# rbitr/llm.f90

Hardware: AMD Instinct MI355X
Metric: tokens/sec TinyLlama-1.1B decode (higher is better)
Workload: dtype f32; 1 GPU; tinyllama f32 decode, greedy, positions 6..1140 (./llm -n 1140 -t 0); consumer=logits to host + host argmax (llmk_forward), parallelism=single GPU, seed=20260928

## Files before the change

### include/llmk.h

```cpp
#ifndef LLMK_H
#define LLMK_H

#include <stddef.h>
#include <stdint.h>

#ifdef __cplusplus
extern "C" {
#endif

#define LLMK_TYPE_F32 0
#define LLMK_TYPE_F16 1
#define LLMK_TYPE_Q4_0 2
#define LLMK_TYPE_Q6_K 14

#define LLMK_TOKEN_EMBEDDING_TABLE 0
#define LLMK_RMS_ATT_WEIGHT 1
#define LLMK_RMS_FFN_WEIGHT 2
#define LLMK_WQKV 3
#define LLMK_WO 4
#define LLMK_W13 5
#define LLMK_W2 6
#define LLMK_RMS_FINAL_WEIGHT 7
#define LLMK_WCLS 8
#define LLMK_N_TENSORS 9

#define LLMK_FLAG_NO_GRAPH 1
#define LLMK_FLAG_TIMINGS 2
#define LLMK_FLAG_MULTI_KERNEL 4

#define LLMK_OK 0
#define LLMK_E_ARG 1
#define LLMK_E_SHAPE 2
#define LLMK_E_SIZE 3
#define LLMK_E_TYPE 4
#define LLMK_E_STATE 5
#define LLMK_E_NODEVICE 6
#define LLMK_E_NOMEM 7
#define LLMK_E_TIMEOUT 8
#define LLMK_E_COMM 9
#define LLMK_E_VERIFY 10
#define LLMK_E_NONFINITE 11
#define LLMK_E_HIP 1000

// ... 30 lines not shown
int llmk_tp_read_partial(llmk_ctx *ctx, float *out);
int llmk_tp_write_partial(llmk_ctx *ctx, const float *in);
int llmk_tp_read_logits(llmk_ctx *ctx, float *out_slice);

int llmk_upload(llmk_ctx *ctx, int tensor_id, const void *host, size_t nbytes, int ggml_type);

int llmk_upload_rows(llmk_ctx *ctx, int tensor_id, int layer, int row_offset, int rows, const void *host,
                     size_t nbytes, int ggml_type);

int llmk_set_tensor_type(llmk_ctx *ctx, int tensor_id, int ggml_type);
int llmk_set_rms_eps(llmk_ctx *ctx, float eps);

int llmk_set_rope_freqs(llmk_ctx *ctx, const float *freqs, int n);

int llmk_forward(llmk_ctx *ctx, int token, int pos, float *logits_out);

int llmk_prefill(llmk_ctx* ctx, const int* tokens, int n, int pos0, float* logits_out);

int llmk_score(llmk_ctx *ctx, const int *tokens, int n, int pos0, const int *targets, float *logprob_out, int *argmax_out,
               float *logits_out);

int llmk_forward_greedy(llmk_ctx *ctx, int token, int pos, int *next_token);

typedef void (*llmk_token_fn)(int index, int token, void *user);
int llmk_decode_greedy(llmk_ctx *ctx, int token, int pos0, int n, int *ids_out, llmk_token_fn on_token, void *user);

int llmk_forward_sample(llmk_ctx *ctx, int token, int pos, float temperature, uint64_t seed, int *next_token);
int llmk_decode_sample(llmk_ctx *ctx, int token, int pos0, int n, float temperature, uint64_t seed,
                       int *ids_out, llmk_token_fn on_token, void *user);

// ... 103 lines not shown
```

### llm.f90_amd/csrc/llmk.hip

```cpp
#include "../../include/llmk.h"
#include "kernels.h"
#include "token_kernel.h"
#include "prefill.h"
#include "batch.h"
#include "tp_p2p.h"

#include <rccl/rccl.h>

#include <algorithm>
#include <vector>

#include <float.h>
#include <math.h>
#include <stdio.h>
#include <stdlib.h>
#include <string.h>
#include <new>

using namespace llmk;

extern "C" int llmk_create_tp(const llmk_config* cfg, int tp_rank, int tp_size, llmk_ctx** out);
static int q16_build(llmk_ctx* c);

#define HIPCHK(expr)                                          \
// ... 62 lines not shown
    unsigned* d_tp_bad = nullptr;
    TpPeers peers = {};
    void* ipc_mapped[TP_MAX_RANKS] = {};
    bool p2p = false;
    float* d_part = nullptr;
    TensorDesc gdesc[LLMK_N_TENSORS];
    TensorDesc desc[LLMK_N_TENSORS];
    DevTensor t[LLMK_N_TENSORS];
    float *d_kc = nullptr, *d_vc = nullptr;
    float *d_x = nullptr, *d_q = nullptr, *d_xb = nullptr, *d_hb = nullptr, *d_logits = nullptr, *d_rope = nullptr;
    int *d_tokpos = nullptr, *d_next = nullptr;
    int* h_tokpos = nullptr;
    float* h_logits = nullptr;
    float* h_logits_dev = nullptr;
    bool tk_direct = true;
    TkNext* h_next = nullptr;
    TkDevWords* dev_words() const { return tk_words_behind<TkDevWords>(d_logits, V); }
    TkHostWords* host_words() const { return tk_words_behind<TkHostWords>(h_logits, V); }
    TkHostWords* host_words_dev() const { return tk_words_behind<TkHostWords>(h_logits_dev, V); }
    hipStream_t stream = nullptr;
    hipGraphExec_t graph[TAIL_COUNT][2] = {};
    llmk_sample_params* h_samp = nullptr;
    DevShadow<llmk_sample_params> samp_dev = {{}, true};
    llmk_filter_params* h_filt = nullptr;
    DevShadow<llmk_filter_params> filt_dev;
    int* d_hist = nullptr;
    int* d_pen_cnt = nullptr;
    llmk_penalty_params* d_pen = nullptr;
    llmk_penalty_params* h_pen = nullptr;
    llmk_logprob_record *d_lp = nullptr, *h_lp = nullptr;
// ... 265 lines not shown
    }
    return launch_gemv_t<EPI_STORE, true>(c->t[LLMK_WCLS].type, c->stream, a, c->n_cu);
}
hipError_t launch_embed(llmk_ctx* c) {
    hipLaunchKernelGGL(embed_kernel, dim3((c->E + 255) / 256), dim3(256), 0, c->stream,
                       (const float*)c->t[LLMK_TOKEN_EMBEDDING_TABLE].data, c->d_tokpos, c->d_x, c->E);
    return hipGetLastError();
}

#define HIPRET(expr)                     \
    do {                                 \
        hipError_t e_ = (expr);          \
        if (e_ != hipSuccess) return e_; \
    } while (0)

struct TkGreedy { int gflags = 0, id_index = 0; };
template <class TK>
hipError_t launch_token_kernel_t(llmk_ctx* c, bool direct, const TkGreedy& g) {
    TokenArgs a;
    a.gflags = g.gflags | ((TK_DEBUG && getenv("LLMK_TK_NOSYNC")) ? TKG_NOSYNC : 0);
    a.emb = (const float*)c->t[LLMK_TOKEN_EMBEDDING_TABLE].data;
    a.rms = (const float*)c->t[LLMK_RMS_ATT_WEIGHT].data;
    a.wqkv = TK::Q4 ? c->q16[LLMK_WQKV] : c->t[LLMK_WQKV].data;
    a.wo = TK::Q4 ? c->q16[LLMK_WO] : c->t[LLMK_WO].data;
    a.w13 = TK::Q4 ? c->q16[LLMK_W13] : c->t[LLMK_W13].data;
    a.w2 = TK::Q4 ? c->q16[LLMK_W2] : c->t[LLMK_W2].data;
    a.wcls = (TK::Q4 && !TK::CLSQ6) ? c->q16[LLMK_WCLS] : c->t[LLMK_WCLS].data;
    a.kc = c->d_kc;
    a.vc = c->d_vc;
    a.rope = c->d_rope;
    a.tokpos = (direct || g.gflags) ? nullptr : c->d_tokpos;
    a.tok_imm = (g.gflags & TKG_CAND_IN) ? g.id_index : c->h_tokpos[0];
    a.pos_imm = c->h_tokpos[1];
    a.serial_imm = c->h_tokpos[2];
    a.g_qkv = c->d_gran;
    a.logits = direct ? c->h_logits_dev : c->d_logits;
    a.err = &c->dev_words()->err;
    a.herr = (direct || g.gflags) ? &c->host_words_dev()->err : nullptr;
    a.zeros = c->d_zeros;
#ifdef LLMK_TK_DEBUG
    a.trace = c->d_trace;
#endif
    a.L = c->L;
    a.S = c->S;
    a.eps = c->eps;
    const dim3 grid((TK_DEBUG && c->tk_short_grid) ? TK_NCU - 1 : TK_NCU);
    if (g.gflags) hipLaunchKernelGGL((token_kernel<TK, true>), grid, dim3(TK_THREADS), c->tk_lds, c->stream, a);
    else hipLaunchKernelGGL((token_kernel<TK>), grid, dim3(TK_THREADS), c->tk_lds, c->stream, a);
    return hipGetLastError();
}
#ifndef LLMK_TK_EXTRA_SHAPES
#define LLMK_TK_EXTRA_SHAPES(X)
#endif
// ... 39 lines not shown
        return LLMK_OK;
    const size_t lds = ((size_t)TkLds<TK>::ATT_S + 2 * (size_t)c->S * sizeof(float) + 15) & ~(size_t)15;
    c->tk_lds = lds < 96 * 1024 ? 96 * 1024 : lds;
    if (c->tk_lds > 160 * 1024) return LLMK_OK;
    HIPCHK(hipFuncSetAttribute((const void*)token_kernel<TK>, hipFuncAttributeMaxDynamicSharedMemorySize, (int)c->tk_lds));
    HIPCHK(hipFuncSetAttribute((const void*)token_kernel<TK, true>, hipFuncAttributeMaxDynamicSharedMemorySize, (int)c->tk_lds));
    int per_cu = 0;
    HIPCHK(hipOccupancyMaxActiveBlocksPerMultiprocessor(&per_cu, token_kernel<TK>, TK_THREADS, c->tk_lds));
    if (per_cu < 1 || (long long)per_cu * c->n_cu < TK_NCU) return LLMK_OK;
    static_assert(tk_qsc_front<TK>() == (size_t)TK::QKV + 3 * (size_t)TK::E + TK::H + (size_t)TK::NH * (TkAttPlan<TK>::PMAX - 1) * (TK::HS + 2),
                  "tk_qsc_front: the attention parts are TkAttPlan's");
    const size_t ngran = tk_qsc_front<TK>() + TK_QSC_GRANULES;
    c->tk_ngran = ngran;
    if (!c->d_gran) HIPCHK(dev_alloc(&c->d_gran, ngran * sizeof(unsigned long long)));
    if (!c->d_zeros) HIPCHK(dev_alloc(&c->d_zeros, (size_t)TK_NCU * TK_WAVES * 1024));
    if (TK_DEBUG && getenv("LLMK_TK_TRACE")) HIPCHK(dev_alloc(&c->d_trace, (size_t)TK_NCU * TK_TRACE_N * 8));
    HIPCHK(hipMemset(c->d_gran, 0, ngran * sizeof(unsigned long long)));
    HIPCHK(hipMemset(c->d_zeros, 0, (size_t)TK_NCU * TK_WAVES * 1024));
    c->use_tk = true;
    c->tk_shape = id;
    return LLMK_OK;
}

int tk_setup_all(llmk_ctx* c) {
    if ((c->cfg.flags & (LLMK_FLAG_MULTI_KERNEL | LLMK_FLAG_TIMINGS)) || c->n_cu != TK_NCU || c->tp_size != 1 || c->tk_retired) return LLMK_OK;
    int rc = LLMK_OK;
    for (int i = 0; i < TK_NSHAPES && rc == LLMK_OK; ++i) rc = tk_table[i].setup(c, i + 1);
    return rc;
}

__global__ void bump_serial_kernel(int* tokpos) { tokpos[2] += 1; }
// ... 173 lines not shown
            if (g) { hipGraphExecDestroy(g); g = nullptr; }
}
int build_graph(llmk_ctx* c, TailMode tail, hipGraphExec_t* out) {
    hipGraph_t g = nullptr;
    HIPCHK(hipStreamBeginCapture(c->stream, hipStreamCaptureModeThreadLocal));
    hipError_t e = enqueue_token(c, tail, false);
    hipError_t e2 = hipStreamEndCapture(c->stream, &g);
    if (e != hipSuccess) { if (g) hipGraphDestroy(g); return LLMK_E_HIP + (int)e; }
    HIPCHK(e2);
    e = hipGraphInstantiate(out, g, nullptr, nullptr, 0);
    hipGraphDestroy(g);
    HIPCHK(e);
    return LLMK_OK;
}

int check_ready(llmk_ctx* c) {
    if (!c) return LLMK_E_ARG;
    for (int i = 0; i < LLMK_N_TENSORS; ++i)
        if (!c->t[i].uploaded) return LLMK_E_STATE;
    if (c->use_tk && tk_table[c->tk_shape - 1].q4 && c->q16_dirty) return q16_build(c);
    return LLMK_OK;
}

constexpr int TK_RANGE_LIMIT = 4;
bool tk_inject_timeout(int pos) {
    const char* at = TK_DEBUG ? getenv("LLMK_TK_INJECT_TIMEOUT") : nullptr;
    return at && atoi(at) == pos;
}
int tk_clear_err(llmk_ctx* c) {
    HIPCHK(hipMemsetAsync(&c->dev_words()->err, 0, sizeof(unsigned), c->stream));
    HIPCHK(hipStreamSynchronize(c->stream));
    c->host_words()->err = 0;
// ... 83 lines not shown
            return LLMK_OK;
        }
        rc = tk_retire(c, err, pos);
        if (rc) return rc;
    }
    return LLMK_E_TIMEOUT;
}
int run_token(llmk_ctx* c, int token, int pos, TailMode tail) {
    const bool filt = tail == TAIL_FILTER || tail == TAIL_PENALTY, samp = tail == TAIL_SAMPLE;
    if (filt) c->filt_dev.invalidate();
    if (samp) c->samp_dev.invalidate();
    const int rc = run_token_pass(c, token, pos, tail);
    if (rc == LLMK_OK && filt) c->filt_dev.confirm(*c->h_filt);
    if (rc == LLMK_OK && samp) c->samp_dev.confirm(*c->h_samp);
    return rc;
}

#ifndef LLMK_PF_H_STEP1
#define LLMK_PF_H_STEP1 1.00
#define LLMK_PF_H_STEP2 1.32
#define LLMK_PF_HQ_STEP1 1.20
#define LLMK_PF_HQ_STEP2 1.92
#endif
struct PfPlan { int nr, nk, total, U, grid; };
PfPlan pf_plan(const llmk_ctx* c, int rows, int K, int T = PF_TMAX, int wt = -1) {
    if (wt < 0) wt = c->cfg.weight_type;
    static const double step_f32[2] = {2.45, 4.25}, step_h[2] = {LLMK_PF_H_STEP1, LLMK_PF_H_STEP2}, step_hq[2] = {LLMK_PF_HQ_STEP1, LLMK_PF_HQ_STEP2};
    static const double step_q8[2] = {LLMK_PF_HQ_STEP1, LLMK_PF_HQ_STEP2 * 0.925};
    static const double step_q6[2] = {LLMK_PF_HQ_STEP1 * 1.3, LLMK_PF_HQ_STEP2 * 1.3};
    const bool q6 = wt == LLMK_TYPE_Q6_K;
// ... 396 lines not shown
    HIPCHK(hipMemsetAsync(c->pf_flag, 0, sizeof(unsigned), c->stream));
    HIPCHK(hipStreamSynchronize(c->stream));
    pf_teardown(c);
    c->pf_hm = false;
    int rc = pf_setup(c);
    if (rc) return rc;
    rc = again();
    if (!for_good) pf_teardown(c);
    return rc;
}

}

extern "C" {

int llmk_version(void) { return 406; }

const char* llmk_strerror(int code) {
    switch (code) {
        case LLMK_OK: return "ok";
        case LLMK_E_ARG: return "llmk: bad argument";
        case LLMK_E_SHAPE: return "llmk: unsupported model shape";
        case LLMK_E_SIZE: return "llmk: byte count does not match tensor size";
        case LLMK_E_TYPE: return "llmk: unsupported ggml tensor type";
        case LLMK_E_STATE: return "llmk: forward called before all weights were uploaded";
        case LLMK_E_NODEVICE: return "llmk: no usable HIP device (there is no CPU fallback)";
        case LLMK_E_NOMEM: return "llmk: out of memory";
        case LLMK_E_TIMEOUT: return "llmk: device-side exchange timed out (persistent kernel not fully resident?)";
        case LLMK_E_COMM: return "llmk: tensor-parallel communicator missing or RCCL error";
        case LLMK_E_VERIFY: return "llmk: uploaded weights did not arrive intact on the device (three attempts)";
        case LLMK_E_NONFINITE: return "llmk: no finite logit at this position (the greedy or sampled pick has no answer)";
// ... 82 lines not shown
    CK(dev_alloc(&c->d_vc, kvn * sizeof(float)));
    CK(dev_alloc(&c->d_x, (size_t)E * sizeof(float)));
    CK(dev_alloc(&c->d_q, (size_t)E * sizeof(float)));
    CK(dev_alloc(&c->d_xb, (size_t)E * sizeof(float)));
    CK(dev_alloc(&c->d_hb, (size_t)H * sizeof(float)));
    CK(dev_alloc(&c->d_part, (size_t)E * sizeof(float)));
    const size_t logits_bytes = (size_t)V * sizeof(float) + sizeof(TkDevWords);
    CK(dev_alloc(&c->d_logits, logits_bytes));
    CK(dev_alloc(&c->d_rope, (size_t)(hs / 2) * sizeof(float)));
    CK(dev_alloc(&c->d_tokpos, 4 * sizeof(int)));
    CK(dev_alloc(&c->d_next, 2 * sizeof(int)));
    CK(hipHostMalloc(&c->h_tokpos, 4 * sizeof(int), hipHostMallocDefault));
    CK(hipHostMalloc(&c->h_logits, (size_t)V * sizeof(float) + sizeof(TkHostWords) + (size_t)S * sizeof(int), hipHostMallocMapped));
    CK(hipHostGetDevicePointer((void**)&c->h_logits_dev, c->h_logits, 0));
    c->tk_direct = !(getenv("LLMK_TK_DIRECT") && getenv("LLMK_TK_DIRECT")[0] == '0');
    CK(hipHostMalloc(&c->h_next, sizeof(TkNext), hipHostMallocDefault));
    CK(hipHostMalloc(&c->h_samp, sizeof(llmk_sample_params), hipHostMallocDefault));
    CK(hipHostMalloc(&c->h_filt, sizeof(llmk_filter_params), hipHostMallocDefault));
    CK(hipStreamCreateWithFlags(&c->stream, hipStreamNonBlocking));
    for (int i = 0; i < 8; ++i) CK(hipEventCreate(&c->ev[i]));
    if (rc == LLMK_OK) rc = tk_setup_all(c);
    if (rc == LLMK_OK) {
        g_prepare = true;
        hipError_t pe = launch_qkv(c, 0);
        if (pe == hipSuccess) pe = launch_attn(c, 0);
        if (pe == hipSuccess) pe = launch_wo(c, 0);
        if (pe == hipSuccess) pe = launch_w13(c, 0);
        if (pe == hipSuccess) pe = launch_w2(c, 0);
        if (pe == hipSuccess) pe = launch_cls(c);
        g_prepare = false;
// ... 220 lines not shown
        if (rc) return rc;
    }
    return LLMK_OK;
}

int llmk_upload_rows(llmk_ctx* c, int tid, int layer, int row_offset, int rows, const void* host, size_t nbytes,
                     int ggml_type) {
    if (!c || !host || tid < 0 || tid >= LLMK_N_TENSORS) return LLMK_E_ARG;
    const TensorDesc& g = c->gdesc[tid];
    DevTensor& t = c->t[tid];
    const int nl = g.layered ? c->L : 1;
    if (layer < 0 || layer >= nl || row_offset < 0 || rows <= 0 || row_offset + rows > g.rows) return LLMK_E_ARG;
    if (ggml_type != t.type) return LLMK_E_TYPE;
    if (nbytes != (size_t)rows * row_bytes_for(ggml_type, g.K)) return LLMK_E_SIZE;
    HIPCHK(hipSetDevice(c->cfg.device));
    if (c->tp_size > 1) return upload_rows_sharded(c, tid, layer, row_offset, rows, (const uint8_t*)host, ggml_type);
    const size_t pitch = row_bytes_for(ggml_type, g.K);
    return upload_block(c, tid, layer, row_offset, rows, (const uint8_t*)host, pitch, 0, pitch);
}

int llmk_upload(llmk_ctx* c, int tid, const void* host, size_t nbytes, int ggml_type) {
    if (!c || !host || tid < 0 || tid >= LLMK_N_TENSORS) return LLMK_E_ARG;
    const TensorDesc& g = c->gdesc[tid];
    const int nl = g.layered ? c->L : 1;
    if (ggml_type != c->t[tid].type) return LLMK_E_TYPE;
    const size_t per_layer = (size_t)g.rows * row_bytes_for(ggml_type, g.K);
    if (nbytes != per_layer * nl) return LLMK_E_SIZE;
    c->t[tid].rows_uploaded = 0;
    c->t[tid].uploaded = false;
    for (int l = 0; l < nl; ++l) {
        int rc = llmk_upload_rows(c, tid, l, 0, g.rows, (const char*)host + (size_t)l * per_layer, per_layer, ggml_type);
        if (rc) return rc;
    }
    return LLMK_OK;
}

int llmk_set_tensor_type(llmk_ctx* c, int tid, int ggml_type) {
    if (!c || tid != LLMK_WCLS) return LLMK_E_ARG;
    if (ggml_type != LLMK_TYPE_F32 && ggml_type != LLMK_TYPE_F16 && ggml_type != LLMK_TYPE_Q4_0 && ggml_type != LLMK_TYPE_Q6_K) return LLMK_E_TYPE;
    DevTensor& t = c->t[tid];
    if (t.type == ggml_type) return LLMK_OK;
    const TensorDesc& d = c->desc[tid];
    const int kalign = ggml_type == LLMK_TYPE_Q6_K ? Q6K_WEIGHTS : ggml_type == LLMK_TYPE_Q4_0 ? 32 : ggml_type == LLMK_TYPE_F16 ? 8 : 4;
    if (d.K % kalign) return LLMK_E_SHAPE;
    HIPCHK(hipSetDevice(c->cfg.device));
    HIPCHK(hipStreamSynchronize(c->stream));
    if (t.data) HIPCHK(hipFree(t.data));
    if (c->pf_ready) pf_teardown(c);
    t.data = nullptr;
    t.type = ggml_type;
    t.uploaded = false;
    t.rows_uploaded = 0;
    const size_t rows = (size_t)d.rows * (d.layered ? c->L : 1);
    t.row_bytes = dev_row_bytes(ggml_type, d.K);
    HIPCHK(dev_alloc(&t.data, rows * t.row_bytes + TENSOR_SLACK));
    HIPCHK(hipMemset(t.data, 0, rows * t.row_bytes + TENSOR_SLACK));
    if (c->q16[tid]) { HIPCHK(hipFree(c->q16[tid])); c->q16[tid] = nullptr; }
    c->q16_dirty = true;
    if (c->use_tk) {
        c->use_tk = false;
        drop_graphs(c);
    }
    { const int rc = tk_setup_all(c); if (rc) return rc; }
    g_prepare = true;
    const hipError_t pe = launch_cls(c);
    g_prepare = false;
    if (pe == hipErrorInvalidValue) return LLMK_E_SHAPE;
    HIPCHK(pe);
    return LLMK_OK;
}

int llmk_set_rms_eps(llmk_ctx* c, float eps) {
    if (!c || !(eps > 0.f) || !(eps < 1.f)) return LLMK_E_ARG;
    HIPCHK(hipSetDevice(c->cfg.device));
    HIPCHK(hipStreamSynchronize(c->stream));
    c->eps = eps;
    drop_graphs(c);
    return LLMK_OK;
}

int llmk_set_rope_freqs(llmk_ctx* c, const float* freqs, int n) {
    if (!c || !freqs || n != c->hs / 2) return LLMK_E_ARG;
    HIPCHK(hipSetDevice(c->cfg.device));
    HIPCHK(hipMemcpy(c->d_rope, freqs, (size_t)n * sizeof(float), hipMemcpyHostToDevice));
    return LLMK_OK;
}

int llmk_forward(llmk_ctx* c, int token, int pos, float* logits_out) {
    if (!c || !logits_out) return LLMK_E_ARG;
    int rc = run_token(c, token, pos, TAIL_LOGITS);
    if (rc) return rc;
    memcpy(logits_out, c->h_logits, (size_t)c->V * sizeof(float));
    return LLMK_OK;
}

int llmk_prefill(llmk_ctx* c, const int* tokens, int n, int pos0, float* logits_out) {
    if (!c || !tokens || !logits_out || n < 1 || pos0 < 1 || pos0 + n - 1 > c->S) return LLMK_E_ARG;
    int rc = check_ready(c);
    if (rc) return rc;
    for (int i = 0; i < n; ++i)
        if (tokens[i] < 1 || tokens[i] > c->V) return LLMK_E_ARG;
    if (!pf_eligible(c)) {
        for (int i = 0; i < n; ++i) {
            rc = run_token(c, tokens[i], pos0 + i, TAIL_LOGITS);
            if (rc) return rc;
        }
        memcpy(logits_out, c->h_logits, (size_t)c->V * sizeof(float));
// ... 272 lines not shown
                if (on_token) on_token(done, ids_out[done], user);
                ++done;
                continue;
            }
            const hipError_t q = hipStreamQuery(c->stream);
            if (q == hipSuccess) { if (ids[done] == 0) break; continue; }
            if (q != hipErrorNotReady) return LLMK_E_HIP + (int)q;
        }
        HIPCHK(hipStreamSynchronize(c->stream));
        for (; done < n && ids[done] != 0; ++done) {
            ids_out[done] = ids[done];
            if (on_token) on_token(done, ids_out[done], user);
        }
        const unsigned err = c->h_next->err;
        if (err == 0 && done == n) {
            for (int i = 0; lp && i < n; ++i) logprob_deliver(c, lp, i, pos0 + i - 1);
            return LLMK_OK;
        }
        rc = tk_range_only(err) ? tk_clear_err(c) : tk_retire(c, err, pos0 + done);
        if (rc) return rc;
        if (done > 0) token = ids_out[done - 1];
        c->tk_short_grid = false;
    }
    for (int i = done; i < n; ++i) {
        rc = run_token(c, token, pos0 + i, tail);
        if (rc) return rc;
        if (c->h_next->id < 1 || c->h_next->id > c->V) return LLMK_E_NONFINITE;
        token = ids_out[i] = c->h_next->id;
        if (lp) c->h_lp[pos0 + i - 1] = c->h_lp[c->S];
        if (on_token) on_token(i, token, user);
// ... 107 lines not shown
    *c->h_lp_top = (unsigned)top_n;
    HIPCHK(hipMemcpyAsync(c->d_logits, logits, (size_t)c->V * sizeof(float), hipMemcpyHostToDevice, c->stream));
    HIPCHK(copy_logprob_top(c));
    HIPCHK(enqueue_logprob(c, c->d_logits, nullptr, nullptr, 0, token, c->d_lp + c->S));
    HIPCHK(hipMemcpyAsync(c->h_lp + c->S, c->d_lp + c->S, sizeof(llmk_logprob_record), hipMemcpyDeviceToHost, c->stream));
    HIPCHK(hipStreamSynchronize(c->stream));
    logprob_deliver(c, &lp, 0, c->S);
    return LLMK_OK;
}
int llmk_set_history(llmk_ctx* c, const int* tokens, int n, int pos0) {
    if (!c || !tokens || n < 1 || pos0 < 1 || pos0 + n - 1 > c->S) return LLMK_E_ARG;
    for (int i = 0; i < n; ++i)
        if (tokens[i] < 0 || tokens[i] > c->V) return LLMK_E_ARG;
    const int rc = pen_setup(c);
    if (rc) return rc;
    HIPCHK(hipMemcpyAsync(c->d_hist + (pos0 - 1), tokens, (size_t)n * sizeof(int), hipMemcpyHostToDevice, c->stream));
    HIPCHK(hipStreamSynchronize(c->stream));
    return LLMK_OK;
}
int llmk_get_history(llmk_ctx* c, int* tokens_out, int n, int pos0) {
    if (!c || !tokens_out || n < 1 || pos0 < 1 || pos0 + n - 1 > c->S) return LLMK_E_ARG;
    const int rc = pen_setup(c);
    if (rc) return rc;
    HIPCHK(hipMemcpyAsync(tokens_out, c->d_hist + (pos0 - 1), (size_t)n * sizeof(int), hipMemcpyDeviceToHost, c->stream));
    HIPCHK(hipStreamSynchronize(c->stream));
    return LLMK_OK;
}

static_assert(LLMK_MAX_BATCH == PF_TMAX, "a batch's rows are the rows of one prefill pass");
constexpr size_t bd_attn_smem(int hs) { return ((size_t)BD_WAVES * 16 * hs + 2 * BD_WAVES * 16) * sizeof(float); }

static void batch_free(llmk_batch* b) {
    void* dev[] = {b->d_kc, b->d_vc, b->d_rows, b->d_tok, b->d_out, b->d_logits, b->d_po, b->d_pml, b->d_next, b->d_filt, b->d_out2, b->d_err, b->d_ids,
                   b->d_hist, b->d_pen_cnt, b->d_pen, b->d_raw, b->d_lp, b->d_lp_top, b->d_pk, b->d_pv, b->d_first, b->d_colmap, b->d_xpo, b->d_xpml};
    for (void* p : dev)
        if (p) hipFree(p);
    void* host[] = {b->h_rows, b->h_tok, b->h_filt, b->h_out, b->h_err, b->h_pen, b->h_lp, b->h_lp_top, b->h_first, b->h_colmap};
    for (void* p : host)
// ... 503 lines not shown
    if (pe == hipSuccess) pe = hipStreamSynchronize(c->stream);
    float ms = 0.f;
    if (pe == hipSuccess) pe = hipEventElapsedTime(&ms, e0, e1);
    hipEventDestroy(e0);
    if (e1) hipEventDestroy(e1);
    HIPCHK(hipMemsetAsync(c->pf_flag, 0, sizeof(unsigned), c->stream));
    HIPCHK(hipStreamSynchronize(c->stream));
    if (pe != hipSuccess) return LLMK_E_HIP + (int)pe;
    *avg_ms = ms / (float)iters;
    return LLMK_OK;
}

int llmk_reset(llmk_ctx* c) {
    if (!c) return LLMK_E_ARG;
    HIPCHK(hipSetDevice(c->cfg.device));
    const size_t kvn = (size_t)c->L * c->S * c->KVl * sizeof(float);
    HIPCHK(hipMemsetAsync(c->d_kc, 0, kvn, c->stream));
    HIPCHK(hipMemsetAsync(c->d_vc, 0, kvn, c->stream));
    HIPCHK(hipMemsetAsync(&c->dev_words()->err, 0, sizeof(unsigned), c->stream));
    HIPCHK(tk_qsc_clear(c, c->stream));
    if (c->d_hist) {
        HIPCHK(hipMemsetAsync(c->d_hist, 0, (size_t)c->S * sizeof(int), c->stream));
        HIPCHK(hipMemsetAsync(c->d_pen_cnt, 0, (size_t)c->V * sizeof(int), c->stream));
    }
    HIPCHK(hipStreamSynchronize(c->stream));
    c->host_words()->err = 0;
    c->h_next->err = 0;
    for (int i = 0; i < 5; ++i) c->times[i] = 0.f;
    return LLMK_OK;
}
// ... 133 lines not shown
    int rc = check_ready(c);
    if (rc) return -rc;
    if (!pf_shape_ok(c)) return LLMK_CLS_NONE;
    auto setup = [&]() -> int {
        HIPCHK(hipSetDevice(c->cfg.device));
        return pf_setup(c, true);
    };
    if ((rc = setup()) != LLMK_OK) return -rc;
    if (sc_plan(c, rows).R > 0) return LLMK_CLS_GEMM;
    return c->t[LLMK_WCLS].type == LLMK_TYPE_Q6_K ? LLMK_CLS_ROWS : LLMK_CLS_NONE;
}

int llmk_peek(llmk_ctx* c, int which, int layer, int pos, float* out, int n) {
    if (!c || !out || n <= 0) return LLMK_E_ARG;
    HIPCHK(hipSetDevice(c->cfg.device));
    const float* src = nullptr;
    int len = 0;
    switch (which) {
        case 0: src = c->d_x; len = c->E; break;
        case 1: src = c->d_q; len = c->Eq; break;
        case 2: src = c->d_xb; len = c->Eq; break;
        case 3: src = c->d_hb; len = c->Hl; break;
        case 4:
        case 5:
            if (layer < 0 || layer >= c->L || pos < 1 || pos > c->S) return LLMK_E_ARG;
            src = (which == 4 ? c->d_kc : c->d_vc) + ((size_t)layer * c->S + (pos - 1)) * c->KVl;
            len = c->KVl;
            break;
#ifdef LLMK_PF_TRACE
        case 7: src = c->pf[0].HB; len = PF_TMAX * c->H; break;
// ... 294 lines not shown
        if (ncclCommCount(c->comm, &n) != ncclSuccess) return -LLMK_E_COMM;
        return n;
    }
    if (c->p2p) {
        int n = 0;
        for (int r = 0; r < c->tp_size; ++r) n += c->peers.inbox[r] != nullptr;
        return n;
    }
    return 1;
}

int llmk_destroy(llmk_ctx* c) {
    if (!c) return LLMK_E_ARG;
    if (c->n_batches > 0) return LLMK_E_STATE;
    hipSetDevice(c->cfg.device);
    if (c->stream) hipStreamSynchronize(c->stream);
    if (c->comm) ncclCommDestroy(c->comm);
    for (int r = 0; r < TP_MAX_RANKS; ++r)
        if (c->ipc_mapped[r]) hipIpcCloseMemHandle(c->ipc_mapped[r]);
    if (c->d_inbox) hipFree(c->d_inbox);
    if (c->d_tp_bad) hipFree(c->d_tp_bad);
    drop_graphs(c);
    for (int i = 0; i < LLMK_N_TENSORS; ++i) {
        if (c->t[i].data && !c->t[i].alias) hipFree(c->t[i].data);
    }
    pf_teardown(c);
    sc_teardown(c);
    void* dev[] = {c->d_kc, c->d_vc, c->d_x, c->d_q, c->d_xb, c->d_hb, c->d_logits, c->d_rope, c->d_tokpos, c->d_next,
                   c->d_gran, c->d_zeros, c->d_trace, c->d_part, c->d_hist, c->d_pen_cnt, c->d_pen, c->d_lp, c->d_lp_raw};
    for (void* p : dev)
        if (p) hipFree(p);
    for (int b = 0; b < 2; ++b) {
        if (c->up_stage[b]) hipHostFree(c->up_stage[b]);
        if (c->up_tmp[b]) hipFree(c->up_tmp[b]);
        if (c->up_done[b]) hipEventDestroy(c->up_done[b]);
    }
    if (c->up_acc) hipFree(c->up_acc);
    for (int i = 0; i < LLMK_N_TENSORS; ++i)
        if (c->q16[i]) hipFree(c->q16[i]);
    if (c->h_tokpos) hipHostFree(c->h_tokpos);
    if (c->h_logits) hipHostFree(c->h_logits);
    if (c->h_next) hipHostFree(c->h_next);
    if (c->h_samp) hipHostFree(c->h_samp);
    if (c->h_filt) hipHostFree(c->h_filt);
    if (c->h_pen) hipHostFree(c->h_pen);
    if (c->h_lp) hipHostFree(c->h_lp);
    if (c->h_lp_top) hipHostFree(c->h_lp_top);
    for (int i = 0; i < 8; ++i)
        if (c->ev[i]) hipEventDestroy(c->ev[i]);
    if (c->stream) hipStreamDestroy(c->stream);
    delete c;
    return LLMK_OK;
}

}
```

### llm.f90_amd/llmk.py

```python
from __future__ import annotations

import ctypes as C
import os
import subprocess

import numpy as np

_HERE = os.path.dirname(os.path.abspath(__file__))
LIB_PATH = os.environ.get("LLMK_LIB") or os.path.join(_HERE, "csrc", "libllmk.so")

TENSOR_IDS = {
    "token_embedding_table": 0, "rms_att_weight": 1, "rms_ffn_weight": 2, "wqkv": 3, "wo": 4, "w13": 5, "w2": 6,
    "rms_final_weight": 7, "wcls": 8,
}
FLAG_NO_GRAPH, FLAG_TIMINGS, FLAG_MULTI_KERNEL = 1, 2, 4
SYMBOLS = ["llmk_create", "llmk_create_tp", "llmk_tp_unique_id", "llmk_tp_init_comm", "llmk_tp_p2p_handle", "llmk_tp_p2p_connect",
           "llmk_tp_p2p_connect_local", "llmk_tp_p2p_selftest", "llmk_tp_p2p_stress", "llmk_tp_p2p_disable", "llmk_tp_begin", "llmk_tp_segment",
           "llmk_tp_read_partial", "llmk_tp_write_partial", "llmk_tp_read_logits", "llmk_upload", "llmk_upload_rows",
           "llmk_set_rope_freqs", "llmk_set_tensor_type", "llmk_set_rms_eps", "llmk_forward", "llmk_prefill", "llmk_forward_greedy", "llmk_decode_greedy",
           "llmk_forward_sample", "llmk_decode_sample", "llmk_forward_sample_ex", "llmk_decode_sample_ex", "llmk_sample_logits", "llmk_set_history", "llmk_get_history",
           "llmk_forward_sample_pen", "llmk_decode_sample_pen", "llmk_sample_logits_pen", "llmk_forward_sample_lp", "llmk_decode_sample_lp",
           "llmk_logprob_logits", "llmk_score", "llmk_batch_create", "llmk_batch_destroy", "llmk_batch_fork", "llmk_batch_forward",
           "llmk_batch_decode", "llmk_batch_time", "llmk_rows_set_history", "llmk_rows_get_history", "llmk_rows_decode",
           "llmk_rows_sample_logits", "llmk_prefix_set", "llmk_prefix_attach", "llmk_prefix_len", "llmk_reset", "llmk_timings",
           "llmk_time_kernel", "llmk_cls_form", "llmk_peek", "llmk_tensor_checksum", "llmk_path", "llmk_tk_shapes", "llmk_tp_ranks_seen", "llmk_destroy", "llmk_strerror", "llmk_version"]
PATH_NAMES = {0: "multi-kernel (5 launches per layer)", 1: "persistent whole-token kernel",
              2: "tensor-parallel rank: 6 launches per layer + one-shot peer-memory exchanges",
              3: "tensor-parallel rank: eager launches + RCCL collectives", 4: "tensor-parallel rank, collectives not connected"}


TOKEN_FN = C.CFUNCTYPE(None, C.c_int, C.c_int, C.c_void_p)


class LlmkError(RuntimeError):
# ... 87 lines not shown
        L.llmk_tp_p2p_selftest.argtypes = [vp, ci]
        L.llmk_tp_p2p_stress.argtypes = [vp, ci, C.c_uint]
        L.llmk_tp_p2p_disable.argtypes = [vp]
        L.llmk_tensor_checksum.argtypes = [vp, ci, C.POINTER(C.c_ulonglong)]
        L.llmk_tp_begin.argtypes = [vp, ci, ci]
        L.llmk_tp_segment.argtypes = [vp, ci, ci]
        L.llmk_tp_read_partial.argtypes = [vp, cf]
        L.llmk_tp_write_partial.argtypes = [vp, cf]
        L.llmk_tp_read_logits.argtypes = [vp, cf]
        L.llmk_upload.argtypes = [vp, ci, vp, C.c_size_t, ci]
        L.llmk_upload_rows.argtypes = [vp, ci, ci, ci, ci, vp, C.c_size_t, ci]
        L.llmk_set_rope_freqs.argtypes = [vp, cf, ci]
        L.llmk_set_tensor_type.argtypes = [vp, ci, ci]
        L.llmk_set_rms_eps.argtypes = [vp, C.c_float]
        L.llmk_forward.argtypes = [vp, ci, ci, cf]
        L.llmk_prefill.argtypes = [vp, C.POINTER(ci), ci, ci, cf]
        L.llmk_forward_greedy.argtypes = [vp, ci, ci, C.POINTER(ci)]
        L.llmk_decode_greedy.argtypes = [vp, ci, ci, ci, C.POINTER(ci), vp, vp]
        if hasattr(L, "llmk_forward_sample"):
            L.llmk_forward_sample.argtypes = [vp, ci, ci, C.c_float, C.c_uint64, C.POINTER(ci)]
            L.llmk_decode_sample.argtypes = [vp, ci, ci, ci, C.c_float, C.c_uint64, C.POINTER(ci), vp, vp]
        if hasattr(L, "llmk_sample_logits"):
            L.llmk_forward_sample_ex.argtypes = [vp, ci, ci, C.POINTER(Sampler), C.POINTER(ci)]
            L.llmk_decode_sample_ex.argtypes = [vp, ci, ci, ci, C.POINTER(Sampler), C.POINTER(ci), vp, vp]
            L.llmk_sample_logits.argtypes = [vp, cf, ci, C.POINTER(Sampler), C.POINTER(ci), C.POINTER(ci), cf]
        if hasattr(L, "llmk_sample_logits_pen"):
            L.llmk_set_history.argtypes = [vp, C.POINTER(ci), ci, ci]
            L.llmk_get_history.argtypes = [vp, C.POINTER(ci), ci, ci]
            L.llmk_forward_sample_pen.argtypes = [vp, ci, ci, C.POINTER(Sampler), C.POINTER(Penalties), C.POINTER(ci)]
            L.llmk_decode_sample_pen.argtypes = [vp, ci, ci, ci, C.POINTER(Sampler), C.POINTER(Penalties), C.POINTER(ci), vp, vp]
# ... 319 lines not shown

    def tp_read_partial(self) -> np.ndarray:
        out = np.empty(self.shape.emb_dim, np.float32)
        _ck(lib().llmk_tp_read_partial(self._h, out.ctypes.data_as(C.POINTER(C.c_float))))
        return out

    def tp_write_partial(self, v: np.ndarray):
        v = np.ascontiguousarray(v, np.float32)
        _ck(lib().llmk_tp_write_partial(self._h, v.ctypes.data_as(C.POINTER(C.c_float))))

    def tp_read_logits(self) -> np.ndarray:
        out = np.empty(self.V // self.tp_size, np.float32)
        _ck(lib().llmk_tp_read_logits(self._h, out.ctypes.data_as(C.POINTER(C.c_float))))
        return out

    def reset(self):
        _ck(lib().llmk_reset(self._h))

    def timings(self):
        t = (C.c_float * 5)()
        _ck(lib().llmk_timings(self._h, t))
        return list(t)

    def time_kernel(self, kernel: int, iters: int):
        ms, b = C.c_float(0), C.c_double(0)
        _ck(lib().llmk_time_kernel(self._h, kernel, iters, C.byref(ms), C.byref(b)))
        return ms.value, b.value

    def cls_form(self, rows: int) -> int:
        rc = lib().llmk_cls_form(self._h, rows)
# ... 158 lines not shown
```

Measured before the change: 1349 tokens/s.

## Speculatively launch next greedy decode step before caller requests it

Adds a speculation state machine that watches whether the caller keeps feeding back the first-max token of the previous logits at the next position. Once that pattern has held for a few steps, it launches the next token's forward on the GPU right away, writing into double-buffered mapped host logits. The GPU chains further launches from its own argmax. A matching call then adopts the precomputed logits, and a mismatching one drains and discards them with exponential backoff. The aim is to hide host-side logits copying, host argmax and launch latency behind GPU compute. The cost is extra synchronisation paths: every state-changing API must settle in-flight work, and a mispredicted step wastes a full forward.

```diff
diff --git a/include/llmk.h b/include/llmk.h
--- a/include/llmk.h
+++ b/include/llmk.h
@@ -27,6 +27,7 @@
 #define LLMK_FLAG_NO_GRAPH 1
 #define LLMK_FLAG_TIMINGS 2
 #define LLMK_FLAG_MULTI_KERNEL 4
+#define LLMK_FLAG_NO_SPECULATE 8
 
 #define LLMK_OK 0
 #define LLMK_E_ARG 1
@@ -87,6 +88,7 @@
 int llmk_set_rope_freqs(llmk_ctx *ctx, const float *freqs, int n);
 
 int llmk_forward(llmk_ctx *ctx, int token, int pos, float *logits_out);
+int llmk_spec_stats(llmk_ctx *ctx, int out[4]);
 
 int llmk_prefill(llmk_ctx* ctx, const int* tokens, int n, int pos0, float* logits_out);
 
diff --git a/llm.f90_amd/csrc/llmk.hip b/llm.f90_amd/csrc/llmk.hip
--- a/llm.f90_amd/csrc/llmk.hip
+++ b/llm.f90_amd/csrc/llmk.hip
@@ -4,10 +4,13 @@
 #include "prefill.h"
 #include "batch.h"
 #include "tp_p2p.h"
+#include "spec_state.h"
 
 #include <rccl/rccl.h>
 
 #include <algorithm>
+#include <chrono>
+#include <mutex>
 #include <vector>
 
 #include <float.h>
@@ -100,6 +103,14 @@
     float* h_logits = nullptr;
     float* h_logits_dev = nullptr;
     bool tk_direct = true;
+    SpecState spec;
+    bool spec_on = false;
+    bool spec_in_forward = false;
+    float* spec_buf[2] = {nullptr, nullptr};
+    float* spec_buf_dev[2] = {nullptr, nullptr};
+    bool spec_wait_event = false;
+    hipEvent_t spec_ev[2] = {nullptr, nullptr};
+    TkHostWords* spec_words(int b) const { return tk_words_behind<TkHostWords>(spec_buf[b], V); }
     TkNext* h_next = nullptr;
     TkDevWords* dev_words() const { return tk_words_behind<TkDevWords>(d_logits, V); }
     TkHostWords* host_words() const { return tk_words_behind<TkHostWords>(h_logits, V); }
@@ -395,7 +406,7 @@
         if (e_ != hipSuccess) return e_; \
     } while (0)
 
-struct TkGreedy { int gflags = 0, id_index = 0; };
+struct TkGreedy { int gflags = 0, id_index = 0; float* logits_dev = nullptr; };
 template <class TK>
 hipError_t launch_token_kernel_t(llmk_ctx* c, bool direct, const TkGreedy& g) {
     TokenArgs a;
@@ -415,9 +426,9 @@
     a.pos_imm = c->h_tokpos[1];
     a.serial_imm = c->h_tokpos[2];
     a.g_qkv = c->d_gran;
-    a.logits = direct ? c->h_logits_dev : c->d_logits;
+    a.logits = g.logits_dev ? g.logits_dev : direct ? c->h_logits_dev : c->d_logits;
     a.err = &c->dev_words()->err;
-    a.herr = (direct || g.gflags) ? &c->host_words_dev()->err : nullptr;
+    a.herr = g.logits_dev ? &tk_words_behind<TkHostWords>(g.logits_dev, c->V)->err : (direct || g.gflags) ? &c->host_words_dev()->err : nullptr;
     a.zeros = c->d_zeros;
 #ifdef LLMK_TK_DEBUG
     a.trace = c->d_trace;
@@ -487,7 +498,7 @@
     c->tk_ngran = ngran;
     if (!c->d_gran) HIPCHK(dev_alloc(&c->d_gran, ngran * sizeof(unsigned long long)));
     if (!c->d_zeros) HIPCHK(dev_alloc(&c->d_zeros, (size_t)TK_NCU * TK_WAVES * 1024));
-    if (TK_DEBUG && getenv("LLMK_TK_TRACE")) HIPCHK(dev_alloc(&c->d_trace, (size_t)TK_NCU * TK_TRACE_N * 8));
+    if (TK_DEBUG && getenv("LLMK_TK_TRACE") && !c->d_trace) HIPCHK(dev_alloc(&c->d_trace, (size_t)TK_NCU * TK_TRACE_N * 8));
     HIPCHK(hipMemset(c->d_gran, 0, ngran * sizeof(unsigned long long)));
     HIPCHK(hipMemset(c->d_zeros, 0, (size_t)TK_NCU * TK_WAVES * 1024));
     c->use_tk = true;
@@ -691,8 +702,13 @@
     return LLMK_OK;
 }
 
+int spec_settle(llmk_ctx* c);
 int check_ready(llmk_ctx* c) {
     if (!c) return LLMK_E_ARG;
+    if (!c->spec_in_forward) {
+        const int rc = spec_settle(c);
+        if (rc) return rc;
+    }
     for (int i = 0; i < LLMK_N_TENSORS; ++i)
         if (!c->t[i].uploaded) return LLMK_E_STATE;
     if (c->use_tk && tk_table[c->tk_shape - 1].q4 && c->q16_dirty) return q16_build(c);
@@ -806,6 +822,140 @@
     if (rc == LLMK_OK && filt) c->filt_dev.confirm(*c->h_filt);
     if (rc == LLMK_OK && samp) c->samp_dev.confirm(*c->h_samp);
     return rc;
+}
+
+constexpr int SPEC_MAX_DEVICES = 64;
+std::mutex g_spec_mutex;
+llmk_ctx* g_spec_owner[SPEC_MAX_DEVICES] = {};
+void spec_register(llmk_ctx* c, bool in_flight) {
+    const int d = c->cfg.device;
+    if (d < 0 || d >= SPEC_MAX_DEVICES) return;
+    std::lock_guard<std::mutex> lock(g_spec_mutex);
+    if (in_flight) g_spec_owner[d] = c;
+    else if (g_spec_owner[d] == c) g_spec_owner[d] = nullptr;
+}
+bool spec_eligible(const llmk_ctx* c) {
+    return c->spec_on && c->spec_buf[0] && c->spec_buf[1] && c->use_tk && c->tk_direct && !c->tk_retired && c->tp_size == 1 && !c->comm && !c->p2p &&
+           c->lp_top_n < 0 && c->cfg.device < SPEC_MAX_DEVICES && c->tk_shape >= 1 && !tk_table[c->tk_shape - 1].q4;
+}
+int spec_drain(llmk_ctx* c) {
+    HIPCHK(hipSetDevice(c->cfg.device));
+    HIPCHK(hipStreamSynchronize(c->stream));
+    spec_register(c, false);
+    unsigned derr = 0;
+    HIPCHK(hipMemcpy(&derr, &c->dev_words()->err, sizeof(unsigned), hipMemcpyDeviceToHost));
+    const bool raised = derr != 0 || c->spec_words(0)->err != 0 || c->spec_words(1)->err != 0;
+    c->spec_words(0)->err = 0;
+    c->spec_words(1)->err = 0;
+    c->tk_short_grid = false;
+    return raised ? tk_clear_err(c) : LLMK_OK;
+}
+int spec_settle_others(llmk_ctx* c) {
+    const int d = c->cfg.device;
+    if (d < 0 || d >= SPEC_MAX_DEVICES) return LLMK_OK;
+    llmk_ctx* o;
+    {
+        std::lock_guard<std::mutex> lock(g_spec_mutex);
+        o = g_spec_owner[d];
+    }
+    if (!o || o == c) return LLMK_OK;
+    return spec_other(o->spec) ? spec_drain(o) : LLMK_OK;
+}
+int spec_settle(llmk_ctx* c) {
+    const int rc = spec_settle_others(c);
+    if (rc) return rc;
+    return spec_other(c->spec) ? spec_drain(c) : LLMK_OK;
+}
+hipError_t spec_launch(llmk_ctx* c, int pos, bool cand_in, int token) {
+    const int b = pos & 1;
+    TkHostWords* w = c->spec_words(b);
+    w->err = 0;
+    w->ids()[0] = 0;
+    HIPRET(c->samp_dev.push(llmk_sample_params{}, [&] { return hipMemsetAsync(&c->dev_words()->samp, 0, sizeof(llmk_sample_params), c->stream); }));
+    const int tok0 = c->h_tokpos[0], pos0 = c->h_tokpos[1];
+    c->h_tokpos[0] = cand_in ? 0 : token - 1;
+    c->h_tokpos[1] = pos;
+    c->h_tokpos[2] += 1;
+    TkGreedy g;
+    g.gflags = TKG_GREEDY | (cand_in ? TKG_CAND_IN | TKG_ID : 0);
+    g.id_index = 0;
+    g.logits_dev = c->spec_buf_dev[b];
+    c->tk_short_grid = tk_inject_timeout(pos);
+    hipError_t e = launch_token_kernel(c, false, g);
+    if (e == hipSuccess && c->spec_wait_event) e = hipEventRecord(c->spec_ev[b], c->stream);
+    c->h_tokpos[0] = tok0;
+    c->h_tokpos[1] = pos0;
+    return e;
+}
+constexpr double SPEC_WAIT_LIMIT_S = 10.0;
+bool spec_wait_id(llmk_ctx* c, int b, int* id) {
+    volatile int* slot = c->spec_words(b)->ids();
+    const auto t0 = std::chrono::steady_clock::now();
+    while (c->spec_wait_event) {
+        const hipError_t q = hipEventQuery(c->spec_ev[b ^ 1]);
+        if (q == hipSuccess) break;
+        if (q != hipErrorNotReady || std::chrono::duration<double>(std::chrono::steady_clock::now() - t0).count() > SPEC_WAIT_LIMIT_S) return false;
+    }
+    for (;;) {
+        for (int spin = 0; spin < 4096; ++spin) {
+            const int v = *slot;
+            if (v != 0) { *id = v; return true; }
+            __builtin_ia32_pause();
+        }
+        const hipError_t q = hipStreamQuery(c->stream);
+        if (q != hipErrorNotReady) { *id = *slot; return q == hipSuccess && *id != 0; }
+        if (std::chrono::duration<double>(std::chrono::steady_clock::now() - t0).count() > SPEC_WAIT_LIMIT_S) return false;
+    }
+}
+int spec_first_max(const float* z, int V) {
+    float bv = -INFINITY;
+    int bi = -1;
+    for (int i = 0; i < V; ++i)
+        if (z[i] > bv) { bv = z[i]; bi = i; }
+    return bi + 1;
+}
+bool spec_forward_begin(llmk_ctx* c, int token, int pos, float* logits_out, int* rc) {
+    SpecState& s = c->spec;
+    *rc = spec_settle_others(c);
+    if (*rc) return true;
+    const bool args_ok = token >= 1 && token <= c->V && pos >= 1 && pos <= c->S;
+    switch (spec_begin_forward(s, args_ok && spec_eligible(c), token, pos)) {
+        case SPEC_PLAIN: return false;
+        case SPEC_DISCARD: *rc = spec_drain(c); return *rc != LLMK_OK;
+        case SPEC_ADOPT: break;
+    }
+    *rc = LLMK_OK;
+    if (hipSetDevice(c->cfg.device) != hipSuccess) { spec_failed(s, false); *rc = spec_drain(c); return *rc != LLMK_OK; }
+    const int b = pos & 1;
+    bool launched = false;
+    c->h_tokpos[0] = token - 1;
+    c->h_tokpos[1] = pos;
+    if (spec_next_wanted(s)) launched = spec_launch(c, pos + 1, true, 0) == hipSuccess;
+    int id = 0;
+    const bool through = launched ? spec_wait_id(c, b ^ 1, &id) : hipStreamSynchronize(c->stream) == hipSuccess;
+    if (through && c->spec_words(b)->err == 0) {
+        memcpy(logits_out, c->spec_buf[b], (size_t)c->V * sizeof(float));
+        spec_adopted(s, launched, id, c->h_tokpos[2]);
+        if (!spec_in_flight(s)) spec_register(c, false);
+        c->tk_range_run = 0;
+        return true;
+    }
+    spec_failed(s, launched);
+    *rc = spec_drain(c);
+    return *rc != LLMK_OK;
+}
+void spec_forward_end(llmk_ctx* c, int pos) {
+    SpecState& s = c->spec;
+    if (!spec_wants_choice(s) || !spec_eligible(c)) return;
+    const int choice = spec_first_max(c->h_logits, c->V);
+    if (!spec_end_forward(s, pos, choice)) return;
+    if (spec_launch(c, pos + 1, false, choice) == hipSuccess) {
+        spec_armed(s, pos + 1, choice, c->h_tokpos[2]);
+        spec_register(c, true);
+    } else {
+        (void)hipGetLastError();
+        spec_other(s);
+    }
 }
 
 #ifndef LLMK_PF_H_STEP1
@@ -1232,7 +1382,7 @@
 
 extern "C" {
 
-int llmk_version(void) { return 406; }
+int llmk_version(void) { return 407; }
 
 const char* llmk_strerror(int code) {
     switch (code) {
@@ -1345,6 +1495,17 @@
     CK(hipHostMalloc(&c->h_logits, (size_t)V * sizeof(float) + sizeof(TkHostWords) + (size_t)S * sizeof(int), hipHostMallocMapped));
     CK(hipHostGetDevicePointer((void**)&c->h_logits_dev, c->h_logits, 0));
     c->tk_direct = !(getenv("LLMK_TK_DIRECT") && getenv("LLMK_TK_DIRECT")[0] == '0');
+    c->spec_on = !(cfg->flags & (LLMK_FLAG_NO_SPECULATE | LLMK_FLAG_TIMINGS | LLMK_FLAG_NO_GRAPH | LLMK_FLAG_MULTI_KERNEL)) && tp_size == 1 &&
+                 !(getenv("LLMK_SPECULATE") && getenv("LLMK_SPECULATE")[0] == '0');
+    c->spec.S = S;
+    for (int b = 0; b < 2 && c->spec_on; ++b) {
+        const size_t bytes = (size_t)V * sizeof(float) + sizeof(TkHostWords) + 16;
+        CK(hipHostMalloc(&c->spec_buf[b], bytes, hipHostMallocMapped));
+        if (rc == LLMK_OK) memset(c->spec_buf[b], 0, bytes);
+        CK(hipHostGetDevicePointer((void**)&c->spec_buf_dev[b], c->spec_buf[b], 0));
+    }
+    c->spec_wait_event = c->spec_on && getenv("LLMK_SPEC_WAIT") && !strcmp(getenv("LLMK_SPEC_WAIT"), "event");
+    for (int b = 0; b < 2 && c->spec_wait_event; ++b) CK(hipEventCreateWithFlags(&c->spec_ev[b], hipEventDisableTiming));
     CK(hipHostMalloc(&c->h_next, sizeof(TkNext), hipHostMallocDefault));
     CK(hipHostMalloc(&c->h_samp, sizeof(llmk_sample_params), hipHostMallocDefault));
     CK(hipHostMalloc(&c->h_filt, sizeof(llmk_filter_params), hipHostMallocDefault));
@@ -1595,6 +1756,7 @@
     if (ggml_type != t.type) return LLMK_E_TYPE;
     if (nbytes != (size_t)rows * row_bytes_for(ggml_type, g.K)) return LLMK_E_SIZE;
     HIPCHK(hipSetDevice(c->cfg.device));
+    { const int src = spec_settle(c); if (src) return src; }
     if (c->tp_size > 1) return upload_rows_sharded(c, tid, layer, row_offset, rows, (const uint8_t*)host, ggml_type);
     const size_t pitch = row_bytes_for(ggml_type, g.K);
     return upload_block(c, tid, layer, row_offset, rows, (const uint8_t*)host, pitch, 0, pitch);
@@ -1625,6 +1787,7 @@
     const int kalign = ggml_type == LLMK_TYPE_Q6_K ? Q6K_WEIGHTS : ggml_type == LLMK_TYPE_Q4_0 ? 32 : ggml_type == LLMK_TYPE_F16 ? 8 : 4;
     if (d.K % kalign) return LLMK_E_SHAPE;
     HIPCHK(hipSetDevice(c->cfg.device));
+    { const int src = spec_settle(c); if (src) return src; }
     HIPCHK(hipStreamSynchronize(c->stream));
     if (t.data) HIPCHK(hipFree(t.data));
     if (c->pf_ready) pf_teardown(c);
@@ -1654,6 +1817,7 @@
 int llmk_set_rms_eps(llmk_ctx* c, float eps) {
     if (!c || !(eps > 0.f) || !(eps < 1.f)) return LLMK_E_ARG;
     HIPCHK(hipSetDevice(c->cfg.device));
+    { const int src = spec_settle(c); if (src) return src; }
     HIPCHK(hipStreamSynchronize(c->stream));
     c->eps = eps;
     drop_graphs(c);
@@ -1663,15 +1827,27 @@
 int llmk_set_rope_freqs(llmk_ctx* c, const float* freqs, int n) {
     if (!c || !freqs || n != c->hs / 2) return LLMK_E_ARG;
     HIPCHK(hipSetDevice(c->cfg.device));
+    { const int src = spec_settle(c); if (src) return src; }
     HIPCHK(hipMemcpy(c->d_rope, freqs, (size_t)n * sizeof(float), hipMemcpyHostToDevice));
     return LLMK_OK;
 }
 
 int llmk_forward(llmk_ctx* c, int token, int pos, float* logits_out) {
     if (!c || !logits_out) return LLMK_E_ARG;
-    int rc = run_token(c, token, pos, TAIL_LOGITS);
-    if (rc) return rc;
+    int rc = LLMK_OK;
+    if (spec_forward_begin(c, token, pos, logits_out, &rc)) return rc;
+    c->spec_in_forward = true;
+    rc = run_token(c, token, pos, TAIL_LOGITS);
+    c->spec_in_forward = false;
+    if (rc) { spec_other(c->spec); return rc; }
     memcpy(logits_out, c->h_logits, (size_t)c->V * sizeof(float));
+    spec_forward_end(c, pos);
+    return LLMK_OK;
+}
+
+int llmk_spec_stats(llmk_ctx* c, int out[4]) {
+    if (!c || !out) return LLMK_E_ARG;
+    for (int i = 0; i < 4; ++i) out[i] = c->spec.stats[i];
     return LLMK_OK;
 }
 
@@ -1974,6 +2150,7 @@
         }
         const unsigned err = c->h_next->err;
         if (err == 0 && done == n) {
+            c->tk_range_run = 0;
             for (int i = 0; lp && i < n; ++i) logprob_deliver(c, lp, i, pos0 + i - 1);
             return LLMK_OK;
         }
@@ -2111,6 +2288,7 @@
         if (tokens[i] < 0 || tokens[i] > c->V) return LLMK_E_ARG;
     const int rc = pen_setup(c);
     if (rc) return rc;
+    { const int src = spec_settle(c); if (src) return src; }
     HIPCHK(hipMemcpyAsync(c->d_hist + (pos0 - 1), tokens, (size_t)n * sizeof(int), hipMemcpyHostToDevice, c->stream));
     HIPCHK(hipStreamSynchronize(c->stream));
     return LLMK_OK;
@@ -2119,6 +2297,7 @@
     if (!c || !tokens_out || n < 1 || pos0 < 1 || pos0 + n - 1 > c->S) return LLMK_E_ARG;
     const int rc = pen_setup(c);
     if (rc) return rc;
+    { const int src = spec_settle(c); if (src) return src; }
     HIPCHK(hipMemcpyAsync(tokens_out, c->d_hist + (pos0 - 1), (size_t)n * sizeof(int), hipMemcpyDeviceToHost, c->stream));
     HIPCHK(hipStreamSynchronize(c->stream));
     return LLMK_OK;
@@ -2652,6 +2831,8 @@
 int llmk_reset(llmk_ctx* c) {
     if (!c) return LLMK_E_ARG;
     HIPCHK(hipSetDevice(c->cfg.device));
+    int rc = spec_settle(c);
+    if (rc) return rc;
     const size_t kvn = (size_t)c->L * c->S * c->KVl * sizeof(float);
     HIPCHK(hipMemsetAsync(c->d_kc, 0, kvn, c->stream));
     HIPCHK(hipMemsetAsync(c->d_vc, 0, kvn, c->stream));
@@ -2815,6 +2996,8 @@
 int llmk_peek(llmk_ctx* c, int which, int layer, int pos, float* out, int n) {
     if (!c || !out || n <= 0) return LLMK_E_ARG;
     HIPCHK(hipSetDevice(c->cfg.device));
+    const int src_rc = spec_settle(c);
+    if (src_rc) return src_rc;
     const float* src = nullptr;
     int len = 0;
     switch (which) {
@@ -3139,6 +3322,8 @@
     if (!c) return LLMK_E_ARG;
     if (c->n_batches > 0) return LLMK_E_STATE;
     hipSetDevice(c->cfg.device);
+    if (c->stream) spec_settle(c);
+    spec_register(c, false);
     if (c->stream) hipStreamSynchronize(c->stream);
     if (c->comm) ncclCommDestroy(c->comm);
     for (int r = 0; r < TP_MAX_RANKS; ++r)
@@ -3165,6 +3350,10 @@
         if (c->q16[i]) hipFree(c->q16[i]);
     if (c->h_tokpos) hipHostFree(c->h_tokpos);
     if (c->h_logits) hipHostFree(c->h_logits);
+    for (float* p : c->spec_buf)
+        if (p) hipHostFree(p);
+    for (hipEvent_t e : c->spec_ev)
+        if (e) hipEventDestroy(e);
     if (c->h_next) hipHostFree(c->h_next);
     if (c->h_samp) hipHostFree(c->h_samp);
     if (c->h_filt) hipHostFree(c->h_filt);
diff --git a/llm.f90_amd/csrc/spec_state.h b/llm.f90_amd/csrc/spec_state.h
--- /dev/null
+++ b/llm.f90_amd/csrc/spec_state.h
@@ -0,0 +1,108 @@
+#ifndef LLMK_SPEC_STATE_H
+#define LLMK_SPEC_STATE_H
+
+namespace llmk {
+
+constexpr int SPEC_BACKOFF_MAX = 64;
+constexpr int SPEC_HITS_TO_ARM = 2;
+constexpr int SPEC_CALM = 8;
+
+enum SpecVerdict { SPEC_PLAIN, SPEC_ADOPT, SPEC_DISCARD };
+enum { SPEC_IDLE, SPEC_PROBING, SPEC_ARMED };
+enum { SPEC_STAT_ARMED, SPEC_STAT_ADOPTED, SPEC_STAT_DISCARDED, SPEC_STAT_PROBED };
+
+struct SpecState {
+    int state = SPEC_IDLE;
+    int S = 0;
+    int last_pos = 0, last_choice = 0;
+    int hits = 0;
+    int fl_pos = 0, fl_token = 0;
+    int fl_serial = 0, fl_parity = 0;
+    int backoff = 1, skip = 0, calm = 0;
+    int stats[4] = {0, 0, 0, 0};
+};
+
+inline void spec_miss(SpecState& s) {
+    s.state = SPEC_IDLE;
+    s.skip = s.backoff;
+    s.backoff = s.backoff * 2 > SPEC_BACKOFF_MAX ? SPEC_BACKOFF_MAX : s.backoff * 2;
+    s.calm = 0;
+    s.hits = 0;
+    s.last_choice = 0;
+}
+
+inline SpecVerdict spec_begin_forward(SpecState& s, bool eligible, int token, int pos) {
+    if (s.state == SPEC_ARMED) {
+        if (eligible && pos == s.fl_pos && token == s.fl_token) return SPEC_ADOPT;
+        ++s.stats[SPEC_STAT_DISCARDED];
+        spec_miss(s);
+        return SPEC_DISCARD;
+    }
+    if (!eligible) {
+        s.state = SPEC_IDLE;
+        s.hits = 0;
+        s.last_choice = 0;
+        return SPEC_PLAIN;
+    }
+    if (s.state == SPEC_PROBING) {
+        if (s.last_choice == 0) return SPEC_PLAIN;
+        if (pos == s.last_pos + 1 && token == s.last_choice) ++s.hits;
+        else spec_miss(s);
+        return SPEC_PLAIN;
+    }
+    if (s.skip > 0) { --s.skip; return SPEC_PLAIN; }
+    s.state = SPEC_PROBING;
+    s.hits = 0;
+    s.last_choice = 0;
+    return SPEC_PLAIN;
+}
+
+inline bool spec_wants_choice(const SpecState& s) { return s.state == SPEC_PROBING; }
+inline bool spec_end_forward(SpecState& s, int pos, int choice) {
+    ++s.stats[SPEC_STAT_PROBED];
+    s.last_pos = pos;
+    s.last_choice = choice;
+    if (choice == 0) { s.hits = 0; return false; }
+    return s.hits >= SPEC_HITS_TO_ARM && pos < s.S;
+}
+inline void spec_armed(SpecState& s, int pos, int token, int serial) {
+    s.state = SPEC_ARMED;
+    s.fl_pos = pos;
+    s.fl_token = token;
+    s.fl_serial = serial;
+    s.fl_parity = pos & 1;
+    ++s.stats[SPEC_STAT_ARMED];
+}
+
+inline bool spec_next_wanted(const SpecState& s) { return s.fl_pos < s.S; }
+inline void spec_adopted(SpecState& s, bool launched, int next_token, int serial) {
+    ++s.stats[SPEC_STAT_ADOPTED];
+    if (++s.calm >= SPEC_CALM) s.backoff = 1;
+    if (launched && next_token != 0) {
+        s.fl_pos += 1;
+        s.fl_token = next_token;
+        s.fl_serial = serial;
+        s.fl_parity = s.fl_pos & 1;
+        return;
+    }
+    s.state = SPEC_IDLE;
+    s.hits = 0;
+    s.last_choice = 0;
+}
+inline void spec_failed(SpecState& s, bool launched) {
+    if (launched) ++s.stats[SPEC_STAT_DISCARDED];
+    spec_miss(s);
+}
+
+inline bool spec_other(SpecState& s) {
+    const bool in_flight = s.state == SPEC_ARMED;
+    if (in_flight) ++s.stats[SPEC_STAT_DISCARDED];
+    if (s.state != SPEC_IDLE) spec_miss(s);
+    return in_flight;
+}
+
+inline int spec_in_flight(const SpecState& s) { return s.state == SPEC_ARMED ? 1 : 0; }
+
+}
+
+#endif
diff --git a/llm.f90_amd/llmk.py b/llm.f90_amd/llmk.py
--- a/llm.f90_amd/llmk.py
+++ b/llm.f90_amd/llmk.py
@@ -13,11 +13,11 @@
     "token_embedding_table": 0, "rms_att_weight": 1, "rms_ffn_weight": 2, "wqkv": 3, "wo": 4, "w13": 5, "w2": 6,
     "rms_final_weight": 7, "wcls": 8,
 }
-FLAG_NO_GRAPH, FLAG_TIMINGS, FLAG_MULTI_KERNEL = 1, 2, 4
+FLAG_NO_GRAPH, FLAG_TIMINGS, FLAG_MULTI_KERNEL, FLAG_NO_SPECULATE = 1, 2, 4, 8
 SYMBOLS = ["llmk_create", "llmk_create_tp", "llmk_tp_unique_id", "llmk_tp_init_comm", "llmk_tp_p2p_handle", "llmk_tp_p2p_connect",
            "llmk_tp_p2p_connect_local", "llmk_tp_p2p_selftest", "llmk_tp_p2p_stress", "llmk_tp_p2p_disable", "llmk_tp_begin", "llmk_tp_segment",
            "llmk_tp_read_partial", "llmk_tp_write_partial", "llmk_tp_read_logits", "llmk_upload", "llmk_upload_rows",
-           "llmk_set_rope_freqs", "llmk_set_tensor_type", "llmk_set_rms_eps", "llmk_forward", "llmk_prefill", "llmk_forward_greedy", "llmk_decode_greedy",
+           "llmk_set_rope_freqs", "llmk_set_tensor_type", "llmk_set_rms_eps", "llmk_forward", "llmk_spec_stats", "llmk_prefill", "llmk_forward_greedy", "llmk_decode_greedy",
            "llmk_forward_sample", "llmk_decode_sample", "llmk_forward_sample_ex", "llmk_decode_sample_ex", "llmk_sample_logits", "llmk_set_history", "llmk_get_history",
            "llmk_forward_sample_pen", "llmk_decode_sample_pen", "llmk_sample_logits_pen", "llmk_forward_sample_lp", "llmk_decode_sample_lp",
            "llmk_logprob_logits", "llmk_score", "llmk_batch_create", "llmk_batch_destroy", "llmk_batch_fork", "llmk_batch_forward",
@@ -135,6 +135,8 @@
         L.llmk_set_tensor_type.argtypes = [vp, ci, ci]
         L.llmk_set_rms_eps.argtypes = [vp, C.c_float]
         L.llmk_forward.argtypes = [vp, ci, ci, cf]
+        if hasattr(L, "llmk_spec_stats"):
+            L.llmk_spec_stats.argtypes = [vp, C.POINTER(ci)]
         L.llmk_prefill.argtypes = [vp, C.POINTER(ci), ci, ci, cf]
         L.llmk_forward_greedy.argtypes = [vp, ci, ci, C.POINTER(ci)]
         L.llmk_decode_greedy.argtypes = [vp, ci, ci, ci, C.POINTER(ci), vp, vp]
@@ -484,6 +486,11 @@
         _ck(lib().llmk_tp_read_logits(self._h, out.ctypes.data_as(C.POINTER(C.c_float))))
         return out
 
+    def spec_stats(self) -> dict:
+        out = (C.c_int * 4)()
+        _ck(lib().llmk_spec_stats(self._h, out))
+        return dict(zip(("armed", "adopted", "discarded", "probed"), (int(v) for v in out)))
+
     def reset(self):
         _ck(lib().llmk_reset(self._h))
 
```

After: 1372 tokens/s (median of 5 runs). +1.7%, better.
